# mehta-lab/VisCy

Hardware: AMD Instinct MI355X
Metric: training patches/sec (Z=5, 256x256, 1->2ch UNeXt2) (higher is better)
Workload: dtype bf16; 1 GPU; UNeXt2 2.5D convnextv2_tiny Z=5 256x256 1->2ch, fwd+MixedLoss(0.5,0,0.5)+bwd+AdamW; per_gpu_batch=512, global_batch=512, parallelism=dp1

## Files before the change

### include/vsx.h

```cpp
#ifndef VSX_H
#define VSX_H
#include <stddef.h>
#include <stdint.h>

#ifdef __cplusplus
extern "C" {
#endif

typedef void* vsx_stream_t;

#define VSX_F32 0
#define VSX_BF16 1

int32_t vsx_version(void);
const char* vsx_last_error(void);
const char* vsx_last_kernel(void);
int32_t vsx_set_flag(const char* name, int32_t value);
int32_t vsx_get_flag(const char* name);
int32_t vsx_det_workspace(float* ws, int64_t floats);
int32_t vsx_det_scope(int32_t on);
int32_t vsx_det_active(void);

#define VSX_A_ROWS 0
#define VSX_A_PATCH2 1
// ... 13 lines not shown
typedef struct VsxGemm {
  const void* A;
  const void* B;
  void* C;
  int32_t M, N, K;
  int32_t lda, ldb, ldc;
  int32_t a_mode, gh, gw, cs;
  int32_t nz;
  int32_t a_coff[8];
  int32_t b_off[8];
  int32_t c_coff[8];
  int32_t c_mode;
  int32_t c_cs;
  int32_t pro;
  const float* grn_s;
  const float* grn_b;
  int32_t hw;
  int32_t epi;
  const float* bias;
  const void* res;
  int32_t ldr;
  const void* aux;
  int32_t ldx;
  float* red0;
  float* red1;
  float* colsum;
  void* C2;
  int64_t b_bstride;
  const float* rscale;
} VsxGemm;

int32_t vsx_gemm_nt(const VsxGemm* p, int32_t dtype, vsx_stream_t stream);
int32_t vsx_gemm_nt_ln_bwd_supported(int64_t M, int32_t N, int32_t K, int32_t dtype);
int32_t vsx_gemm_tn(const VsxGemm* p, int32_t dtype, vsx_stream_t stream);

typedef struct VsxGemmPlan {
  const char* family;
  int32_t esize;
  int32_t tile[2];
  int32_t step;
  int32_t nbuf;
  int32_t pro_kind;
  int32_t tr;
  int32_t epi;
  int32_t grid[3], block;
  int32_t pro_bits;
  int64_t zero_c, zero_colsum;
  int64_t det_floats;
} VsxGemmPlan;
#define VSX_GEMM_NT 0
#define VSX_GEMM_TN 1
int32_t vsx_gemm_plan(int32_t kind, const VsxGemm* p, int32_t dtype, VsxGemmPlan* out);



int32_t vsx_dwconv7_fwd(const void* x, const float* w, const float* bias, const void* add, void* y,
    int32_t B, int32_t H, int32_t W, int32_t C, int32_t dtype, vsx_stream_t stream);

int32_t vsx_dwconv7_bwd_data(const void* dy, const float* w, const void* add, void* dx, int32_t B, int32_t H,
    int32_t W, int32_t C, int32_t dtype, vsx_stream_t stream);

int32_t vsx_dwconv7_bwd_weight(const void* dy, const void* x, float* dw, float* db, float* ws,
    int32_t ws_rows, int32_t B, int32_t H, int32_t W, int32_t C, int32_t dtype, vsx_stream_t stream);

int32_t vsx_head_conv_supported(int32_t H2, int32_t W2, int32_t c3, int32_t cmid, int32_t zo, int32_t dtype);
int64_t vsx_head_conv_det_floats(int32_t B, int32_t H2, int32_t W2);
// ... 354 lines not shown
```

### viscy_amd/_lib.py

```python

from __future__ import annotations

import ctypes as C
import os

import torch

_HERE = os.path.dirname(os.path.abspath(__file__))
LIB_PATH = os.environ.get("VSX_LIB", os.path.join(_HERE, "libvsx.so"))

VSX_F32, VSX_BF16 = 0, 1
A_ROWS, A_PATCH2, A_CONV3 = 0, 1, 2
PRO_NONE, PRO_GRN = 0, 1
EPI_NONE, EPI_BIAS, EPI_BIAS_GELU_SQ, EPI_BIAS_RES, EPI_DZ, EPI_BIAS_STATS, EPI_LN_BWD = 0, 1, 2, 3, 4, 5, 6
LOSS_SLOTS, LOSS_SLOT_STRIDE = 64, 32
SPOTLIGHT_CHUNK = 16384
SPOTLIGHT_THRESHOLD, SPOTLIGHT_MASK_U8, SPOTLIGHT_MASK_F32 = 0, 1, 2
SPOTLIGHT_WS_FWD, SPOTLIGHT_WS_OTSU = 0, 1

_I32, _F32, _P, _I64 = C.c_int32, C.c_float, C.c_void_p, C.c_int64


class VsxGemm(C.Structure):
    _fields_ = [
# ... 15 lines not shown
        ("rscale", _P),
    ]


class VsxGemmPlan(C.Structure):
    _fields_ = [
        ("family", C.c_char_p), ("esize", _I32), ("tile", _I32 * 2), ("step", _I32), ("nbuf", _I32), ("pro_kind", _I32), ("tr", _I32),
        ("epi", _I32), ("grid", _I32 * 3), ("block", _I32), ("pro_bits", _I32), ("zero_c", _I64), ("zero_colsum", _I64),
        ("det_floats", _I64),
    ]


class VsxWTask(C.Structure):
    _fields_ = [("kind", _I32), ("dtype", _I32), ("i0", _I32), ("i1", _I32), ("i2", _I32), ("i3", _I32),
                ("p0", _P), ("p1", _P), ("p2", _P), ("p3", _P), ("p4", _P), ("p5", _P), ("p6", _P), ("p7", _P)]


WTASK_PREP, WTASK_TRANSPOSE, WTASK_MATVEC, WTASK_MLP_PACK, WTASK_UNPREP, WTASK_MATVEC_T, WTASK_REDUCE_ROWS = 0, 1, 2, 3, 4, 5, 6

_SIGS = {
    "vsx_version": (_I32, []),
    "vsx_weight_tasks": (_I32, [_P, _I32, _P]),
    "vsx_last_error": (C.c_char_p, []),
    "vsx_last_kernel": (C.c_char_p, []),
    "vsx_set_flag": (_I32, [C.c_char_p, _I32]),
    "vsx_get_flag": (_I32, [C.c_char_p]),
    "vsx_det_workspace": (_I32, [_P, _I64]),
    "vsx_det_scope": (_I32, [_I32]),
    "vsx_det_active": (_I32, []),
    "vsx_gemm_nt": (_I32, [C.POINTER(VsxGemm), _I32, _P]),
    "vsx_gemm_tn": (_I32, [C.POINTER(VsxGemm), _I32, _P]),
    "vsx_gemm_plan": (_I32, [_I32, C.POINTER(VsxGemm), _I32, C.POINTER(VsxGemmPlan)]),
    "vsx_gemm_nt_ln_bwd_supported": (_I32, [_I64, _I32, _I32, _I32]),
    "vsx_ln_fwd": (_I32, [_P, _P, _P, _P, _P, _P, _I32, _I32, _F32, _I32, _P]),
    "vsx_ln_bwd": (_I32, [_P, _P, _P, _P, _P, _P, _P, _P, _P, _I32, _I32, _I32, _P]),
    "vsx_grn_scale": (_I32, [_P, _P, _P, _I32, _I32, _F32, _P]),
    "vsx_grn_bwd_stats": (_I32, [_P, _P, _P, _P, _P, _P, _P, _P, _I32, _I32, _F32, _P]),
    "vsx_grn_gelu_bwd": (_I32, [_P, _P, _P, _P, _P, _P, _I32, _I32, _I32, _I32, _I32, _P]),
    "vsx_dwconv7_fwd": (_I32, [_P, _P, _P, _P, _P, _I32, _I32, _I32, _I32, _I32, _P]),
    "vsx_dwconv7_bwd_data": (_I32, [_P, _P, _P, _P, _I32, _I32, _I32, _I32, _I32, _P]),
    "vsx_dwconv7_bwd_weight": (_I32, [_P, _P, _P, _P, _P, _I32, _I32, _I32, _I32, _I32, _I32, _P]),
    "vsx_stem_im2col": (_I32, [_P, _P, _P, _P, _I32, _I32, _I32, _I32, _I32, _I32, _I32, _I32, _I32, _P]),
    "vsx_stem_im2col_ld": (_I32, [_P, _P, _P, _P, _I32, _I32, _I32, _I32, _I32, _I32, _I32, _I32, _I32, _I32, _P]),
    "vsx_pad_cols": (_I32, [_P, _P, _I32, _I32, _I32, _I32, _P]),
    "vsx_im2col3x3": (_I32, [_P, _P, _I32, _I32, _I32, _I32, _I32, _P]),
    "vsx_col2im3x3": (_I32, [_P, _P, _I32, _I32, _I32, _I32, _I32, _P]),
    "vsx_pixel_shuffle_cat_fwd": (_I32, [_P, _P, _P, _I32, _I32, _I32, _I32, _I32, _I32, _P]),
    "vsx_pixel_shuffle_cat_bwd": (_I32, [_P, _P, _P, _I32, _I32, _I32, _I32, _I32, _I32, _P]),
    "vsx_head_shuffle_fwd": (_I32, [_P, _P, _I32, _I32, _I32, _I32, _I32, _I32, _I32, _P]),
    "vsx_head_shuffle_bwd": (_I32, [_P, _P, _I32, _I32, _I32, _I32, _I32, _I32, _I32, _P]),
    "vsx_head_out_fwd": (_I32, [_P] * 7 + [_I32] * 6 + [_F32, _I32, _P]),
    "vsx_head_out_bwd1": (_I32, [_P] * 11 + [_I32] * 6 + [_F32, _I32, _P]),
    "vsx_head_out_bwd1_wgrad": (_I32, [_P] * 13 + [_I32] * 6 + [_F32, _I32, _P]),
    "vsx_head_out_bwd2": (_I32, [_P] * 9 + [_I32] * 6 + [_F32, _I32, _P]),
    "vsx_loss_pool": (_I32, [_P] * 7 + [_I32] * 3 + [_P]),
    "vsx_ssim_scale_fwd": (_I32, [_P] * 5 + [_I32] * 5 + [_P]),
    "vsx_ssim_scale_bwd": (_I32, [_P] * 7 + [_I32] * 5 + [_F32, _F32, _P, _I32, _P]),
    "vsx_loss_finalize": (_I32, [_P] * 5 + [_F32, _I32, _I32, _I32, _F32, _F32, _F32, _P, _P, _P, _P, _P]),
    "vsx_ssim_scale_fwd_dmu": (_I32, [_P] * 6 + [_I32] * 6 + [_P]),
    "vsx_ssim_scale_bwd_in": (_I32, [_P] * 6 + [_I32] * 5 + [_F32, _F32, _P, _I32, _I32, _P]),
    "vsx_loss_tmax": (_I32, [_P, _I64, _P, _P]),
    "vsx_ssim_scale_fwd_fused": (_I32, [_P] * 11 + [_I32] * 6 + [_P]),
    "vsx_adamw": (_I32, [_P, _P, _P, _P, _P, _I64, _P]),
    "vsx_adamw_advance": (_I32, [_P, _P, _P, _P]),
    "vsx_fill_f32": (_I32, [_P, _I64, _F32, _P]),
    "vsx_mlp_supported": (_I32, [_I32, _I32, _I64, _I32]),
# ... 163 lines not shown
```

### viscy_amd/csrc/gemm.hip

```cpp
#include "vsx_common.h"
#include "../../include/vsx.h"

typedef __attribute__((ext_vector_type(4))) float f32x4;
typedef __attribute__((ext_vector_type(8))) __bf16 bf16x8;
typedef __attribute__((ext_vector_type(4))) short s16x4;

bool vsx_gemm_nt2_ok(const VsxGemm* p);
bool vsx_gemm_nt2_lnbwd_ok(const VsxGemm* p);
void vsx_gemm_nt2_plan(const VsxGemm* p, VsxGemmPlan& pl);
int vsx_gemm_nt2_run(const VsxGemmPlan& pl, const VsxGemm* p, hipStream_t s);

struct RowCoord {
  int b, y, x;
  bool valid;
};

__device__ __forceinline__ RowCoord decode_row(const VsxGemm& p, int m) {
  RowCoord r;
  r.valid = m < p.M;
  int mm = r.valid ? m : 0;
  if (p.a_mode == VSX_A_ROWS && p.c_mode == VSX_A_ROWS) {
    r.b = p.hw > 0 ? mm / p.hw : 0;
    r.y = 0;
    r.x = mm;
// ... 830 lines not shown
  NT_FAST2(T, VSX_EPI_BIAS_RES, BK, NBUF) NT_FAST2(T, VSX_EPI_DZ, BK, NBUF)
  switch (inst_key(pl)) {
    NT_GEN(bf16_t, 128, 2, 2, 128)
    NT_GEN(bf16_t, 128, 2, 2, 32) NT_GEN(float, 128, 2, 2, 32)
    NT_GEN(bf16_t, 64, 2, 2, 32) NT_GEN(float, 64, 2, 2, 32)
    NT_GEN(bf16_t, 32, 4, 1, 32) NT_GEN(float, 32, 4, 1, 32)
    NT_GEN(bf16_t, 16, 4, 1, 32) NT_GEN(float, 16, 4, 1, 32)
    NT_FAST(bf16_t, 64, 1)
    NT_FAST(bf16_t, 64, 2)
    NT_FAST(bf16_t, 32, 1)
    NT_FAST(bf16_t, 32, 2) NT_FAST(float, 32, 2)
    default: vsx_set_error("vsx_gemm_nt: the plan names no instantiation"); return 1;
  }
#undef NT_GEN
#undef NT_FAST1
#undef NT_FAST2
#undef NT_FAST
  VSX_LAUNCH_CHECK();
  g_vsx_last_kernel = pl.family;
  return 0;
}

extern "C" int32_t vsx_gemm_nt(const VsxGemm* p, int32_t dtype, vsx_stream_t stream) {
  VsxGemmPlan pl;
  if (int e = plan_nt(p, dtype, pl)) return e;
  return run_nt(pl, p, reinterpret_cast<hipStream_t>(stream));
}

extern "C" int32_t vsx_gemm_nt_ln_bwd_supported(int64_t M, int32_t N, int32_t K, int32_t dtype) {
  if (dtype != VSX_BF16 || M <= 0 || M >= (1ll << 31)) return 0;
  VsxGemm q = {};
  q.M = (int32_t)M; q.N = N; q.K = K; q.lda = K; q.ldb = K; q.ldc = N; q.a_mode = VSX_A_ROWS; q.c_mode = VSX_A_ROWS; q.epi = VSX_EPI_LN_BWD;
  return vsx_gemm_nt2_lnbwd_ok(&q) ? 1 : 0;
}

template <bool TR>
__device__ __forceinline__ bf16x8 lds_frag_mn_bf16(const char* tile, int LDB, int col0, int p16, int kq) {
  if (TR) {
    const int q = p16;
    const char* a0 = tile + (kq * 4 + (q >> 2)) * LDB + (col0 + (q & 3) * 4) * 2;
    const char* a1 = a0 + 16 * LDB;
    s16x4 lo = __builtin_amdgcn_ds_read_tr16_b64_v4i16((s16x4 __attribute__((address_space(3)))*)(a0));
    s16x4 hi = __builtin_amdgcn_ds_read_tr16_b64_v4i16((s16x4 __attribute__((address_space(3)))*)(a1));
    union {
      struct { s16x4 lo, hi; } s;
      bf16x8 v;
    } u;
    u.s.lo = lo;
    u.s.hi = hi;
    return u.v;
  } else {
    union {
      unsigned short h[8];
      bf16x8 v;
    } u;
#pragma unroll
    for (int j = 0; j < 8; ++j) {
      int mloc = j < 4 ? kq * 4 + j : 16 + kq * 4 + (j - 4);
      u.h[j] = *reinterpret_cast<const unsigned short*>(tile + mloc * LDB + (col0 + p16) * 2);
    }
    return u.v;
  }
}

template <typename T, bool TR>
__device__ __forceinline__ typename Frag<T>::type lds_frag_mn(const char* tile, int LDB, int col0, int p16, int kq,
// ... 666 lines not shown
```

### viscy_amd/csrc/gemm_nt2.hip

```cpp
#include "vsx_common.h"
#include "../../include/vsx.h"

typedef __attribute__((ext_vector_type(4))) float nt2_f32x4;
typedef __attribute__((ext_vector_type(8))) __bf16 nt2_bf16x8;

namespace {

constexpr int BM = 256, BK = 32, NST = 3;
constexpr int ROWB = BK * 2;
constexpr int CW_LD = 68;
constexpr int CW_BYTES = 16 * CW_LD * 4;
constexpr int RED_OFF = 8 * CW_BYTES;

template <int BN>
struct Nt2Geom {
  static constexpr int FN = BN / 32;
  static constexpr int A_BYTES = BM * ROWB, B_BYTES = BN * ROWB, STAGE = A_BYTES + B_BYTES;
  static constexpr int NPA = (BM / 16) / 8, NPB = (BN / 16) / 8;
  static constexpr int PER_SLAB = NPA + NPB;
  static constexpr int LDS_BYTES = NST * STAGE;
  static constexpr int WAVES_PER_SIMD = BN == 128 ? 4 : 2;
  static_assert(RED_OFF + 8 * 2 * (BN / 2) * 4 <= LDS_BYTES, "epilogue staging overlays the operand stages");
};

template <int EPI, int BN, bool PRO = false>
__global__ __launch_bounds__(512, Nt2Geom<BN>::WAVES_PER_SIMD) void gemm_nt2_kernel(const VsxGemm p) {
  typedef Nt2Geom<BN> G;
  constexpr int FN = G::FN, A_BYTES = G::A_BYTES, STAGE = G::STAGE, WN = BN / 2;
  constexpr int PRO_FLOATS = PRO ? 2 * 3072 : 4;
  __shared__ __attribute__((aligned(1024))) char smem[G::LDS_BYTES];
  __shared__ __attribute__((aligned(16))) float gsb[PRO_FLOATS];
  const int tid = threadIdx.x, lane = tid & 63;
  const int wave = __builtin_amdgcn_readfirstlane(tid >> 6);
  const int wm = wave >> 1, wn = wave & 1;
// ... 261 lines not shown
    }
  }

  if constexpr (REDUCE) {
    if (p.hw % BM == 0) {
      asm volatile("s_waitcnt lgkmcnt(0)" ::: "memory");
      __builtin_amdgcn_s_barrier();
      if (tid < BN && n0 + tid < p.N) {
        const int w0 = tid / WN, c = tid % WN;
        float a0 = 0.f, a1 = 0.f;
#pragma unroll
        for (int w = 0; w < 4; ++w) {
          a0 += red[((w * 2 + w0) * 2 + 0) * WN + c];
          if constexpr (EPI == VSX_EPI_DZ) a1 += red[((w * 2 + w0) * 2 + 1) * WN + c];
        }
        if (EPI == VSX_EPI_BIAS_GELU_SQ && p.aux != nullptr) {
          reinterpret_cast<float*>(const_cast<void*>(p.aux))[(size_t)tile_m * p.N + n0 + tid] = a0;
        } else {
          atomicAdd(p.red0 + (size_t)b_tile * p.N + n0 + tid, a0);
          if constexpr (EPI == VSX_EPI_DZ) atomicAdd(p.red1 + (size_t)b_tile * p.N + n0 + tid, a1);
        }
      }
    }
  }
}

#ifdef NT2_TS
__device__ unsigned long long g_nt2_ts[8 * 80];
#define NT2_STAMP(k) do { if (blockIdx.x == gridDim.x / 2 + 3 && lane == 0) g_nt2_ts[wave * 80 + (k)] = __builtin_amdgcn_s_memtime(); } while (0)
#else
#define NT2_STAMP(k) do { } while (0)
#endif

template <int BN>
__global__ __launch_bounds__(512, 2) void gemm_nt2_lnbwd_kernel(const VsxGemm p) {
  typedef Nt2Geom<BN> G;
  constexpr int FN = BN / 16, A_BYTES = G::A_BYTES, STAGE = G::STAGE, NCG = BN / 64;
  __shared__ __attribute__((aligned(1024))) char smem[G::LDS_BYTES];
  const int tid = threadIdx.x, lane = tid & 63;
  const int wave = __builtin_amdgcn_readfirstlane(tid >> 6);
  const int p16 = lane & 15, kq = lane >> 4;
  int bid = blockIdx.x;
  const int m0 = bid * BM;
  NT2_STAMP(0);

  const int dr = lane >> 2;
  const int dc = (lane & 3) ^ ((lane >> 4) & 2);
  const char* Ab = reinterpret_cast<const char*>(p.A) + (size_t)m0 * (size_t)p.lda * 2;
  const char* Bb = reinterpret_cast<const char*>(p.B);
  uint32_t offA[G::NPA], offB[G::NPB];
#pragma unroll
  for (int i = 0; i < G::NPA; ++i) offA[i] = (uint32_t)((wave + 8 * i) * 16 + dr) * (uint32_t)(p.lda * 2) + dc * 16;
#pragma unroll
  for (int i = 0; i < G::NPB; ++i) {
    int nb = (wave + 8 * i) * 16 + dr;
    nb = nb < p.N ? nb : p.N - 1;
    offB[i] = (uint32_t)nb * (uint32_t)(p.ldb * 2) + dc * 16;
  }
  auto issue = [&](int kt, int st) {
    char* S = smem + st * STAGE;
    const char* Ak = Ab + (size_t)kt * ROWB;
    const char* Bk = Bb + (size_t)kt * ROWB;
#pragma unroll
    for (int i = 0; i < G::NPA; ++i)
      __builtin_amdgcn_global_load_lds((const __attribute__((address_space(1))) void*)(Ak + offA[i]),
                                       (__attribute__((address_space(3))) void*)(S + (wave + 8 * i) * 1024), 16, 0, 0);
#pragma unroll
    for (int i = 0; i < G::NPB; ++i)
      __builtin_amdgcn_global_load_lds((const __attribute__((address_space(1))) void*)(Bk + offB[i]),
                                       (__attribute__((address_space(3))) void*)(S + A_BYTES + (wave + 8 * i) * 1024), 16, 0, 0);
// ... 16 lines not shown
    for (int jg = 0; jg < FN; jg += 4) {
      nt2_bf16x8 bf[4];
#pragma unroll
      for (int j = 0; j < 4; ++j) bf[j] = *reinterpret_cast<const nt2_bf16x8*>(S + fragB + (jg + j) * 16 * ROWB);
#pragma unroll
      for (int i = 0; i < 2; ++i)
#pragma unroll
        for (int j = 0; j < 4; ++j)
          acc[i][jg + j] = __builtin_amdgcn_mfma_f32_16x16x32_bf16(af[i], bf[j], acc[i][jg + j], 0, 0, 0);
    }
  };

  const int nk = p.K / BK;
  constexpr int er_ = 0;
  const int erow = lane >> 3, ecol = (lane & 7) * 8;
  const bf16_t* XHp = reinterpret_cast<const bf16_t*>(p.aux);
  uint4 xpre[2][NCG][2];
  float mupre[2][2], rspre[2][2];
  auto prefetch_pass = [&](int i) {
#pragma unroll
    for (int h = 0; h < 2; ++h) {
      const int m = m0 + wave * 32 + i * 16 + erow + 8 * h;
      mupre[i][h] = p.grn_b ? p.grn_b[m] : 0.f;
      rspre[i][h] = p.grn_s[m];
#pragma unroll
      for (int cg = 0; cg < NCG; ++cg) {
        const int n = cg * 64 + ecol;
        xpre[i][cg][h] = n < p.N ? ldvec<bf16_t>(XHp + (size_t)m * p.ldx + n) : make_uint4(0u, 0u, 0u, 0u);
      }
    }
  };
  auto prefetch_rows = [&]() { prefetch_pass(0); };
  (void)er_;
  issue(0, 0);
  if (nk > 1) issue(1, 1);
  if (nk < 3) prefetch_rows();
  int st = 0, stn = NST - 1;
  for (int kt = 0; kt < nk; ++kt) {
    if (kt + 1 < nk) {
      if constexpr (G::PER_SLAB == 3) asm volatile("s_waitcnt vmcnt(3)" ::: "memory");
      else asm volatile("s_waitcnt vmcnt(4)" ::: "memory");
    } else {
      asm volatile("s_waitcnt vmcnt(0)" ::: "memory");
    }
    __builtin_amdgcn_s_barrier();
    if (kt < 64) NT2_STAMP(8 + kt);
    if (kt + 2 < nk) issue(kt + 2, stn);
    if (kt == nk - 3) prefetch_rows();
    compute(st);
    st = st == NST - 1 ? 0 : st + 1;
    stn = stn == NST - 1 ? 0 : stn + 1;
  }
  NT2_STAMP(1);
  asm volatile("s_waitcnt lgkmcnt(0)" ::: "memory");
  __builtin_amdgcn_s_barrier();
  NT2_STAMP(2);

  float* Cw = reinterpret_cast<float*>(smem + wave * CW_BYTES);
  const int er = lane >> 3, ec = (lane & 7) * 8;
  const float invC = 1.f / (float)p.N;
  const bf16_t* XH = reinterpret_cast<const bf16_t*>(p.aux);
  bf16_t* DY = reinterpret_cast<bf16_t*>(p.C);
  const float* MEAN = p.grn_b;
#pragma unroll
  for (int i = 0; i < 2; ++i) {
    float v[NCG][2][8];
    uint4 (&xq)[NCG][2] = xpre[i];
    float s1[2] = {0.f, 0.f}, s2[2] = {0.f, 0.f};
#pragma unroll
    for (int cg = 0; cg < NCG; ++cg) {
      const int n = cg * 64 + ec;
      const bool ok = n < p.N;
#pragma unroll
      for (int j = 0; j < 4; ++j)
#pragma unroll
        for (int r = 0; r < 4; ++r) Cw[(kq * 4 + r) * CW_LD + j * 16 + p16] = acc[i][cg * 4 + j][r];
      __builtin_amdgcn_fence(__ATOMIC_RELEASE, "wavefront");
      __builtin_amdgcn_wave_barrier();
#pragma unroll
      for (int h = 0; h < 2; ++h) {
        const float4 t0 = *reinterpret_cast<const float4*>(Cw + (er + 8 * h) * CW_LD + ec);
        const float4 t1 = *reinterpret_cast<const float4*>(Cw + (er + 8 * h) * CW_LD + ec + 4);
        const float t[8] = {t0.x, t0.y, t0.z, t0.w, t1.x, t1.y, t1.z, t1.w};
        float xf[8];
        unpack<bf16_t>(xq[cg][h], xf);
        if (MEAN && ok) {
          const float mu = mupre[i][h], rsd = rspre[i][h];
#pragma unroll
          for (int e = 0; e < 8; ++e) xf[e] = (xf[e] - mu) * rsd;
          xq[cg][h] = pack<bf16_t>(xf);
          unpack<bf16_t>(xq[cg][h], xf);
        }
#pragma unroll
        for (int e = 0; e < 8; ++e) {
          const float d = ok ? round_bf16(t[e]) : 0.f;
          v[cg][h][e] = d;
          s1[h] += d;
          s2[h] = fmaf(d, xf[e], s2[h]);
        }
      }
      __builtin_amdgcn_fence(__ATOMIC_RELEASE, "wavefront");
      __builtin_amdgcn_wave_barrier();
    }
    NT2_STAMP(3 + i);
    if (i == 0) prefetch_pass(1);
#pragma unroll
    for (int h = 0; h < 2; ++h) {
      s1[h] += __shfl_xor(s1[h], 1, 64); s1[h] += __shfl_xor(s1[h], 2, 64); s1[h] += __shfl_xor(s1[h], 4, 64);
      s2[h] += __shfl_xor(s2[h], 1, 64); s2[h] += __shfl_xor(s2[h], 2, 64); s2[h] += __shfl_xor(s2[h], 4, 64);
      const int m = m0 + wave * 32 + i * 16 + er + 8 * h;
      const float rs = MEAN ? 1.f : rspre[i][h];
      const float m1 = s1[h] * invC, m2 = s2[h] * invC;
#pragma unroll
      for (int cg = 0; cg < NCG; ++cg) {
        const int n = cg * 64 + ec;
        if (n < p.N) {
          float xf[8], o[8];
          unpack<bf16_t>(xq[cg][h], xf);
#pragma unroll
          for (int e = 0; e < 8; ++e) o[e] = rs * (v[cg][h][e] - m1 - xf[e] * m2);
          stvec<bf16_t>(DY + (size_t)m * p.ldc + n, pack<bf16_t>(o));
        }
      }
    }
  }
  NT2_STAMP(5);
}

int pick_bn(int N) {
  if (g_vsx_nt2 & 4) return 128;
  int best = 128, best_cost = 1 << 30;
  for (int bn = 128; bn <= ((g_vsx_nt2 & 8) ? 256 : 384); bn += 128) {
    const int tiles = (N + bn - 1) / bn;
    if (3 * (tiles * bn - N) > N && bn != 128) continue;
    const int cost = tiles * (BM + bn);
    if (cost < best_cost) { best_cost = cost; best = bn; }
  }
  return best;
}

}

bool vsx_gemm_nt2_lnbwd_ok(const VsxGemm* p) {
  return p->a_mode == VSX_A_ROWS && p->c_mode == VSX_A_ROWS && p->pro == VSX_PRO_NONE && p->nz <= 1 && p->K % BK == 0 &&
         p->M % BM == 0 && p->N >= 64 && p->N <= 256 && p->N % 8 == 0 && p->b_bstride == 0 &&
         (unsigned long long)BM * p->lda * 2 < (1ull << 32) && (unsigned long long)p->N * p->ldb * 2 < (1ull << 32);
}

bool vsx_gemm_nt2_ok(const VsxGemm* p) {
  if (p->epi == VSX_EPI_LN_BWD) return vsx_gemm_nt2_lnbwd_ok(p);
  if (!(g_vsx_nt2 & 1)) return false;
  if (p->a_mode != VSX_A_ROWS || p->c_mode != VSX_A_ROWS || p->nz > 1) return false;
  if (p->pro != VSX_PRO_NONE) {
    if (p->pro != VSX_PRO_GRN || p->hw <= 0 || p->hw % BM != 0 || p->K > 3072) return false;
    if (p->epi != VSX_EPI_BIAS_RES && p->epi != VSX_EPI_NONE) return false;
  }
// ... 7 lines not shown
  if (g_vsx_nt2 & 2) return true;
  if (vsx_det_on() && p->epi == VSX_EPI_BIAS_GELU_SQ) return true;
  const int bn = pick_bn(p->N);
  if ((long)(p->M / BM) * vsx_cdiv(p->N, bn) < 256) return false;
  if (p->epi == VSX_EPI_DZ) return false;
  if (p->pro == VSX_PRO_GRN) return p->K >= 768 && p->N >= 192;
  if (p->epi == VSX_EPI_BIAS_GELU_SQ) return bn == 384 && p->N % 384 == 0 && p->K >= 384 && p->K <= 768;
  return p->K >= 768 && (p->N > 192 || ((g_vsx_nt2 & 16) && p->N == 192));
}

void vsx_gemm_nt2_plan(const VsxGemm* p, VsxGemmPlan& pl) {
  const bool lnbwd = p->epi == VSX_EPI_LN_BWD;
  const int bn = lnbwd ? (p->N <= 128 ? 128 : 256) : pick_bn(p->N);
  pl.family = "gemm_nt2";
  pl.tile[0] = BM; pl.tile[1] = bn; pl.step = BK; pl.nbuf = NST;
  pl.epi = p->epi;
  pl.pro_kind = p->pro == VSX_PRO_GRN;
  pl.grid[0] = (p->M / BM) * (lnbwd ? 1 : vsx_cdiv(p->N, bn)); pl.grid[1] = pl.grid[2] = 1;
  pl.block = 512;
  if (vsx_det_on() && p->epi == VSX_EPI_BIAS_GELU_SQ && p->hw > 0 && p->hw % BM == 0 && p->hw > BM) pl.det_floats = (long)(p->M / BM) * p->N;
}

int vsx_gemm_nt2_run(const VsxGemmPlan& pl, const VsxGemm* p, hipStream_t s) {
  VsxGemm q = *p;
  float* det_ws;
  if (int e = vsx_det_take("vsx_gemm_nt", pl.det_floats, &det_ws)) return e;
  if (det_ws) q.aux = det_ws;
  const dim3 grid(pl.grid[0]), block(pl.block);
#define NT2(EPI, BN, PRO) case (EPI) << 12 | (BN) << 1 | (PRO): hipLaunchKernelGGL((gemm_nt2_kernel<EPI, BN, PRO>), grid, block, 0, s, q); break;
#define NT2_BN(BN)  \
  NT2(VSX_EPI_NONE, BN, false) NT2(VSX_EPI_BIAS, BN, false) NT2(VSX_EPI_BIAS_GELU_SQ, BN, false) NT2(VSX_EPI_BIAS_RES, BN, false) \
  NT2(VSX_EPI_DZ, BN, false) NT2(VSX_EPI_NONE, BN, true) NT2(VSX_EPI_BIAS_RES, BN, true)
#define NT2_LNBWD(BN) case VSX_EPI_LN_BWD << 12 | (BN) << 1: hipLaunchKernelGGL((gemm_nt2_lnbwd_kernel<BN>), grid, block, 0, s, q); break;
  switch (pl.epi << 12 | pl.tile[1] << 1 | pl.pro_kind) {
    NT2_BN(128)
    NT2_BN(256)
    NT2_BN(384)
    NT2_LNBWD(128)
    NT2_LNBWD(256)
    default: vsx_set_error("vsx_gemm_nt: the plan names no gemm_nt2 instantiation"); return 1;
  }
#undef NT2
#undef NT2_BN
#undef NT2_LNBWD
  VSX_LAUNCH_CHECK();
  g_vsx_last_kernel = pl.family;
  if (det_ws) return vsx_det_group_sum(det_ws, p->N, 0, p->red0, p->M / p->hw, p->hw / BM, p->N, s);
  return 0;
}

#ifdef NT2_TS
extern "C" int32_t vsx_debug_nt2_ts(unsigned long long* host_out) {
  return hipMemcpyFromSymbol(host_out, HIP_SYMBOL(g_nt2_ts), sizeof(g_nt2_ts)) == hipSuccess ? 0 : 1;
}
#endif
```

### viscy_amd/engine_unext2.py

```python

from __future__ import annotations

import os
from collections import namedtuple
from typing import NamedTuple

import torch
from torch import Tensor

from . import _lib as L
from . import ops as hip_ops
from .flat import FlatEngine, engine_apply


class _BlockW:

    __slots__ = ("C", "p", "dw_w", "W1f", "W1fT", "b1f", "W2", "W2T", "v1", "fc2_w", "fc2_b", "grn_w", "grn_b", "dp", "img", "img2", "b2f")


class _ProjW:
    __slots__ = ("cin", "cout", "taps", "ln", "conv", "W", "WT")


FWD_UNFUSED, FWD_PAIR, FWD_FC1 = 0, 1, 2
# ... 740 lines not shown
            B, H, Wd = sv["shape"]
            dev = self.device
            za_key = ("bwd", B, H, Wd, sv["masked"])
            self._za = za = _ZeroArena(dev, self._za_need.get(za_key, 0), self.ops)
            if cfg.get("head") == "embed":
                d = self._embed_tail_bwd(sv, dout[0], dout[1], dt, B)
            elif cfg.get("head", "conv") == "shuffle":
                fh, fw = sv["head"]
                sxy = cfg["stem_kernel"][-1]
                vs = o.voxel_shuffle_bwd
                if (cfg["out_channels"] * cfg["out_stack_depth"] * sxy * sxy) % (8 if dt == torch.bfloat16 else 4):
                    vs = o.narrow_voxel_shuffle_bwd
                d = vs(dout.contiguous().float(), B, fh, fw, cfg["out_channels"], cfg["out_stack_depth"], sxy, True, dt)
            else:
                hdt = self._head_dtype(dt)
                d = self._head_conv_bwd(sv, dout, hdt, B, dev)
                if hdt != dt:
                    d = d.to(dt)
            dskips = {}
            for k in (2, 1, 0) if cfg.get("head") != "embed" else ():
                proj, blocks = W["dec"][k]
                st_sv = sv["dec"][k]
                cat, xn, mean, rstd, c_up, sc = st_sv["proj"]
                _, sh, sw_, _ = (None, *sv["feat_dims"][2 - k])
                Mk, ccat = B * sh * sw_, c_up + sc
                for bw, bsv in zip(reversed(blocks), reversed(st_sv["blocks"])):
                    d = self._block_bwd(d, bw, bsv, B, sh, sw_, dt)
                if proj.cout < 16:
                    dxn = o.narrow_proj_bwd(d, cat, mean, rstd, proj.ln.weight, proj.ln.bias, proj.conv.weight, g(proj.conv.weight),
                                            g(proj.conv.bias), Mk, ccat, proj.cout)
                else:
                    o.gemm("tn", xn, d, g(proj.conv.weight), Mk, proj.cout, ccat, ccat, proj.cout, ccat, dtype=dt,
                           colsum=g(proj.conv.bias))
                    dxn = torch.empty((Mk, ccat), dtype=dt, device=dev)
                    o.gemm("nt", d, proj.WT, dxn, Mk, ccat, proj.cout, proj.cout, proj.cout, ccat, dtype=dt)
                dcat = o.ln_bwd(dxn, cat, mean, rstd, proj.ln.weight, None, g(proj.ln.weight), g(proj.ln.bias), Mk, ccat)
                del dxn
                d, dskips[2 - k] = o.pixel_shuffle_cat_bwd(dcat, B, sh // 2, sw_ // 2, c_up, sc)
                del dcat
                pre = W["dec_pre"][k]
                if pre is not None:
                    pc, _, WpT = pre
                    lh, lw, cpc = sh // 2, sw_ // 2, 4 * c_up
                    Ml = B * lh * lw
                    col = o.im2col3x3(st_sv["pre_in"], B, lh, lw, cpc)
                    dWp = self._za.take(cpc, 9 * cpc)
                    o.gemm("tn", col, d, dWp, Ml, cpc, 9 * cpc, 9 * cpc, cpc, 9 * cpc, dtype=dt, colsum=g(pc.bias))
                    o.unprep_grad(dWp, g(pc.weight), cpc, cpc, 9)
                    del col
                    dcol = torch.empty((Ml, 9 * cpc), dtype=dt, device=dev)
                    o.gemm("nt", d, WpT, dcol, Ml, 9 * cpc, cpc, cpc, cpc, 9 * cpc, dtype=dt)
                    d = o.col2im3x3(dcol, B, lh, lw, cpc)
                    del dcol
            yield from self._segment_end(0)
            if self.encoder_frozen():
                self._za_need[za_key] = za.used
                yield from self._segment_end(1)
                yield from self._segment_end(2)
                return
            for i in (3, 2, 1, 0):
                proj, blocks = W["enc"][i]
                st_sv = sv["enc"][i]
                ch, cw, cc = sv["feat_dims"][i]
                for bw, bsv in zip(reversed(blocks), reversed(st_sv["blocks"])):
                    d = self._block_bwd(d, bw, bsv, B, ch, cw, dt)
                if proj is not None:
                    prev, xn, mean, rstd = st_sv["proj"]
                    cin = proj.cin
                    Mo = B * ch * cw
# ... 49 lines not shown
```

### viscy_amd/ops.py

```python

from __future__ import annotations

import contextlib
import ctypes as C
import os
import threading
from typing import Sequence

import torch
from torch import Tensor

from . import _lib as L
from ._lib import VsxGemm, VsxGemmPlan, check, dtype_code, lib, ptr, stream


class Scratch:

    def __init__(self, alloc=None):
        self._alloc = alloc or (lambda floats, dev: torch.empty(floats, dtype=torch.float32, device=dev))
        self._tls = threading.local()
        self.held: list = []

    def take(self, dev, floats: int):
        arenas = getattr(self._tls, "arenas", None)
# ... 98 lines not shown
    p.grn_s, p.grn_b = ptr(grn_s), ptr(grn_b)
    p.hw = hw
    p.epi = epi
    p.bias, p.res, p.ldr = ptr(bias), ptr(res), ldr
    p.aux, p.ldx = ptr(aux), ldx
    p.red0, p.red1, p.colsum = ptr(red0), ptr(red1), ptr(colsum)
    p.C2 = ptr(C2)
    p.b_bstride = b_bstride
    p.rscale = ptr(rscale)
    if plan is not None:
        return check(lib().vsx_gemm_plan(0 if kind == "nt" else 1, C.byref(p), dtype_code(dtype), C.byref(plan)), f"gemm_plan_{kind}")
    if kind == "nt" and epi == L.EPI_BIAS_GELU_SQ:
        _det(A.device, lambda: _gemm_det_floats(p, dtype))
    fn = lib().vsx_gemm_nt if kind == "nt" else lib().vsx_gemm_tn
    check(fn(C.byref(p), dtype_code(dtype), stream()), f"gemm_{kind}")


def _gemm_det_floats(p: VsxGemm, dtype: torch.dtype) -> int:
    plan = VsxGemmPlan()
    check(lib().vsx_gemm_plan(0, C.byref(p), dtype_code(dtype), C.byref(plan)), "gemm_plan_nt")
    return plan.det_floats


def tn_grn_stats_ok(M: int, N: int, K: int, hw: int, dtype: torch.dtype) -> bool:
    if dtype != torch.bfloat16 or not lib().vsx_get_flag(b"tn_rect") & 8:
        return False
    p = VsxGemm()
    p.A = p.B = p.C = p.grn_s = p.grn_b = p.aux = p.red0 = 1
    p.M, p.N, p.K, p.lda, p.ldb, p.ldc, p.ldx, p.nz, p.pro, p.hw = M, N, K, K, N, K, K, 1, L.PRO_GRN, hw
    return lib().vsx_gemm_plan(1, C.byref(p), L.VSX_BF16, C.byref(VsxGemmPlan())) == 0


def dgrad_ln_bwd(dh: Tensor, WT: Tensor, xh: Tensor, rstd: Tensor, M: int, C: int, K: int,
                 mean: Tensor | None = None) -> Tensor | None:
    if dh.dtype != torch.bfloat16 or not lib().vsx_gemm_nt_ln_bwd_supported(M, C, K, dtype_code(dh.dtype)):
        return None
    dy = torch.empty((M, C), dtype=dh.dtype, device=dh.device)
    gemm("nt", dh, WT, dy, M, C, K, K, K, C, dtype=dh.dtype, epi=L.EPI_LN_BWD, aux=xh, ldx=C, grn_s=rstd, grn_b=mean)
    return dy


def gemm_z(kind: str, *args, nz: int, a_coff, b_off, c_coff, **kw) -> None:
    for s in range(0, nz, 8):
        e = min(nz, s + 8)
        gemm(kind, *args, nz=e - s, a_coff=a_coff[s:e], b_off=b_off[s:e], c_coff=c_coff[s:e], **kw)


def ln_fwd(x: Tensor, gamma: Tensor | None, beta: Tensor | None, rows: int, Cc: int, eps: float = 1e-6,
           need_mean: bool = True):
    y = torch.empty_like(x)
    mean = torch.empty(rows, dtype=torch.float32, device=x.device) if need_mean else None
    rstd = torch.empty(rows, dtype=torch.float32, device=x.device)
    check(lib().vsx_ln_fwd(ptr(x), ptr(y), ptr(mean), ptr(rstd), ptr(gamma), ptr(beta), rows, Cc, eps,
                           dtype_code(x.dtype), stream()), "ln_fwd")
    return y, mean, rstd


def ln_bwd(dy: Tensor, x: Tensor, mean: Tensor | None, rstd: Tensor, gamma: Tensor | None, add: Tensor | None,
           dgamma: Tensor | None, dbeta: Tensor | None, rows: int, Cc: int) -> Tensor:
    dx = torch.empty_like(dy)
    check(lib().vsx_ln_bwd(ptr(dy), ptr(x), ptr(mean), ptr(rstd), ptr(gamma), ptr(add), ptr(dx), ptr(dgamma),
                           ptr(dbeta), rows, Cc, dtype_code(dy.dtype), stream()), "ln_bwd")
    return dx


def grn_scale(colsq: Tensor, gamma: Tensor, eps: float = 1e-6) -> Tensor:
    s = torch.empty_like(colsq)
    check(lib().vsx_grn_scale(ptr(colsq), ptr(gamma), ptr(s), colsq.shape[0], colsq.shape[1], eps, stream()), "grn_scale")
    return s


# ... 1010 lines not shown
```

Measured before the change: 5600 patches/s.

## Fuse affine LayerNorm backward into decoder projection dgrad GEMM epilogue

Adds an affine variant of the NT GEMM LN-backward epilogue that applies gamma, computes the input gradient, and accumulates per-tile dgamma/dbeta partials into a workspace. A row-reduction kernel (or the deterministic group sum) then finishes the partials. The decoder projection backward uses it, avoiding a round trip of the dxn intermediate through memory and a separate ln_bwd launch. In exchange it adds register pressure and LDS staging in the epilogue, two extra small reduction launches, and it falls back to the old path when the shape is unsupported.

```diff
diff --git a/include/vsx.h b/include/vsx.h
--- a/include/vsx.h
+++ b/include/vsx.h
@@ -69,6 +69,7 @@
 
 int32_t vsx_gemm_nt(const VsxGemm* p, int32_t dtype, vsx_stream_t stream);
 int32_t vsx_gemm_nt_ln_bwd_supported(int64_t M, int32_t N, int32_t K, int32_t dtype);
+int64_t vsx_gemm_nt_ln_bwd_affine_ws_floats(int64_t M, int32_t N, int32_t K, int32_t dtype);
 int32_t vsx_gemm_tn(const VsxGemm* p, int32_t dtype, vsx_stream_t stream);
 
 typedef struct VsxGemmPlan {
diff --git a/viscy_amd/_lib.py b/viscy_amd/_lib.py
--- a/viscy_amd/_lib.py
+++ b/viscy_amd/_lib.py
@@ -71,6 +71,7 @@
     "vsx_gemm_tn": (_I32, [C.POINTER(VsxGemm), _I32, _P]),
     "vsx_gemm_plan": (_I32, [_I32, C.POINTER(VsxGemm), _I32, C.POINTER(VsxGemmPlan)]),
     "vsx_gemm_nt_ln_bwd_supported": (_I32, [_I64, _I32, _I32, _I32]),
+    "vsx_gemm_nt_ln_bwd_affine_ws_floats": (_I64, [_I64, _I32, _I32, _I32]),
     "vsx_ln_fwd": (_I32, [_P, _P, _P, _P, _P, _P, _I32, _I32, _F32, _I32, _P]),
     "vsx_ln_bwd": (_I32, [_P, _P, _P, _P, _P, _P, _P, _P, _P, _I32, _I32, _I32, _P]),
     "vsx_grn_scale": (_I32, [_P, _P, _P, _I32, _I32, _F32, _P]),
diff --git a/viscy_amd/csrc/gemm.hip b/viscy_amd/csrc/gemm.hip
--- a/viscy_amd/csrc/gemm.hip
+++ b/viscy_amd/csrc/gemm.hip
@@ -886,6 +886,10 @@
   VsxGemm q = {};
   q.M = (int32_t)M; q.N = N; q.K = K; q.lda = K; q.ldb = K; q.ldc = N; q.a_mode = VSX_A_ROWS; q.c_mode = VSX_A_ROWS; q.epi = VSX_EPI_LN_BWD;
   return vsx_gemm_nt2_lnbwd_ok(&q) ? 1 : 0;
+}
+
+extern "C" int64_t vsx_gemm_nt_ln_bwd_affine_ws_floats(int64_t M, int32_t N, int32_t K, int32_t dtype) {
+  return vsx_gemm_nt_ln_bwd_supported(M, N, K, dtype) ? 2 * (M / 256) * (int64_t)N : 0;
 }
 
 template <bool TR>
diff --git a/viscy_amd/csrc/gemm_nt2.hip b/viscy_amd/csrc/gemm_nt2.hip
--- a/viscy_amd/csrc/gemm_nt2.hip
+++ b/viscy_amd/csrc/gemm_nt2.hip
@@ -1,5 +1,7 @@
 #include "vsx_common.h"
 #include "../../include/vsx.h"
+
+__global__ void reduce_rows_kernel(const float* __restrict__ ws, float* __restrict__ out, int R, int N);
 
 typedef __attribute__((ext_vector_type(4))) float nt2_f32x4;
 typedef __attribute__((ext_vector_type(8))) __bf16 nt2_bf16x8;
@@ -327,10 +329,12 @@
 #define NT2_STAMP(k) do { } while (0)
 #endif
 
-template <int BN>
+template <int BN, int NCG = BN / 64, bool AFF = false>
 __global__ __launch_bounds__(512, 2) void gemm_nt2_lnbwd_kernel(const VsxGemm p) {
   typedef Nt2Geom<BN> G;
-  constexpr int FN = BN / 16, A_BYTES = G::A_BYTES, STAGE = G::STAGE, NCG = BN / 64;
+  constexpr int FN = NCG * 4, A_BYTES = G::A_BYTES, STAGE = G::STAGE;
+  constexpr int GAM_OFF = RED_OFF + 8 * 2 * BN * 4;
+  static_assert(GAM_OFF + BN * 4 <= G::LDS_BYTES, "the affine epilogue's staging overlays the operand stages");
   __shared__ __attribute__((aligned(1024))) char smem[G::LDS_BYTES];
   const int tid = threadIdx.x, lane = tid & 63;
   const int wave = __builtin_amdgcn_readfirstlane(tid >> 6);
@@ -413,6 +417,8 @@
   };
   auto prefetch_rows = [&]() { prefetch_pass(0); };
   (void)er_;
+  float gpre = 1.f;
+  if constexpr (AFF) if (tid < p.N) gpre = p.bias[tid];
   issue(0, 0);
   if (nk > 1) issue(1, 1);
   if (nk < 3) prefetch_rows();
@@ -436,6 +442,11 @@
   asm volatile("s_waitcnt lgkmcnt(0)" ::: "memory");
   __builtin_amdgcn_s_barrier();
   NT2_STAMP(2);
+  float* gam = reinterpret_cast<float*>(smem + GAM_OFF);
+  if constexpr (AFF) {
+    if (tid < BN) gam[tid] = gpre;
+    __syncthreads();
+  }
 
   float* Cw = reinterpret_cast<float*>(smem + wave * CW_BYTES);
   const int er = lane >> 3, ec = (lane & 7) * 8;
@@ -443,15 +454,27 @@
   const bf16_t* XH = reinterpret_cast<const bf16_t*>(p.aux);
   bf16_t* DY = reinterpret_cast<bf16_t*>(p.C);
   const float* MEAN = p.grn_b;
+  float* red = reinterpret_cast<float*>(smem + RED_OFF);
 #pragma unroll
   for (int i = 0; i < 2; ++i) {
-    float v[NCG][2][8];
+    float v[AFF ? 1 : NCG][2][8];
+    uint4 vq[AFF ? NCG : 1][2];
     uint4 (&xq)[NCG][2] = xpre[i];
     float s1[2] = {0.f, 0.f}, s2[2] = {0.f, 0.f};
+    auto load_gamma = [&](int n, float (&gm)[8]) {
+      const float4 g0 = *reinterpret_cast<const float4*>(gam + n), g1 = *reinterpret_cast<const float4*>(gam + n + 4);
+      gm[0] = g0.x; gm[1] = g0.y; gm[2] = g0.z; gm[3] = g0.w; gm[4] = g1.x; gm[5] = g1.y; gm[6] = g1.z; gm[7] = g1.w;
+    };
 #pragma unroll
     for (int cg = 0; cg < NCG; ++cg) {
       const int n = cg * 64 + ec;
       const bool ok = n < p.N;
+      float gm[8], pg[8], pb[8];
+      if constexpr (AFF) {
+        load_gamma(n, gm);
+#pragma unroll
+        for (int e = 0; e < 8; ++e) { pg[e] = 0.f; pb[e] = 0.f; }
+      }
 #pragma unroll
       for (int j = 0; j < 4; ++j)
 #pragma unroll
@@ -464,45 +487,114 @@
         const float4 t1 = *reinterpret_cast<const float4*>(Cw + (er + 8 * h) * CW_LD + ec + 4);
         const float t[8] = {t0.x, t0.y, t0.z, t0.w, t1.x, t1.y, t1.z, t1.w};
         float xf[8];
+        if constexpr (AFF) asm volatile("" : "+v"(xq[cg][h].x), "+v"(xq[cg][h].y), "+v"(xq[cg][h].z), "+v"(xq[cg][h].w));
         unpack<bf16_t>(xq[cg][h], xf);
-        if (MEAN && ok) {
+        if constexpr (AFF) {
+          const float mu = mupre[i][h], rsd = rspre[i][h];
+#pragma unroll
+          for (int e = 0; e < 8; ++e) xf[e] = ok ? (xf[e] - mu) * rsd : 0.f;
+        } else if (MEAN && ok) {
           const float mu = mupre[i][h], rsd = rspre[i][h];
 #pragma unroll
           for (int e = 0; e < 8; ++e) xf[e] = (xf[e] - mu) * rsd;
           xq[cg][h] = pack<bf16_t>(xf);
           unpack<bf16_t>(xq[cg][h], xf);
         }
+        float dq[8];
 #pragma unroll
         for (int e = 0; e < 8; ++e) {
-          const float d = ok ? round_bf16(t[e]) : 0.f;
-          v[cg][h][e] = d;
+          float d = ok ? round_bf16(t[e]) : 0.f;
+          if constexpr (AFF) {
+            pg[e] = fmaf(d, xf[e], pg[e]);
+            pb[e] += d;
+            dq[e] = d;
+            d *= gm[e];
+          } else {
+            v[cg][h][e] = d;
+          }
           s1[h] += d;
           s2[h] = fmaf(d, xf[e], s2[h]);
         }
+        if constexpr (AFF) vq[cg][h] = pack<bf16_t>(dq);
       }
       __builtin_amdgcn_fence(__ATOMIC_RELEASE, "wavefront");
       __builtin_amdgcn_wave_barrier();
+      if constexpr (AFF) {
+        float* Pg = Cw + (er * 2) * CW_LD + ec;
+        *reinterpret_cast<float4*>(Pg) = make_float4(pg[0], pg[1], pg[2], pg[3]);
+        *reinterpret_cast<float4*>(Pg + 4) = make_float4(pg[4], pg[5], pg[6], pg[7]);
+        *reinterpret_cast<float4*>(Pg + CW_LD) = make_float4(pb[0], pb[1], pb[2], pb[3]);
+        *reinterpret_cast<float4*>(Pg + CW_LD + 4) = make_float4(pb[4], pb[5], pb[6], pb[7]);
+        __builtin_amdgcn_fence(__ATOMIC_RELEASE, "wavefront");
+        __builtin_amdgcn_wave_barrier();
+        float a0 = 0.f, a1 = 0.f;
+#pragma unroll
+        for (int r = 0; r < 8; ++r) {
+          a0 += Cw[(r * 2) * CW_LD + lane];
+          a1 += Cw[(r * 2 + 1) * CW_LD + lane];
+        }
+        float* rw = red + (wave * 2) * BN + cg * 64 + lane;
+        if (i == 0) { rw[0] = a0; rw[BN] = a1; }
+        else { rw[0] += a0; rw[BN] += a1; }
+        __builtin_amdgcn_fence(__ATOMIC_RELEASE, "wavefront");
+        __builtin_amdgcn_wave_barrier();
+      }
     }
     NT2_STAMP(3 + i);
-    if (i == 0) prefetch_pass(1);
+    if constexpr (AFF) {
+#pragma unroll
+      for (int cg = 0; cg < NCG; ++cg)
+#pragma unroll
+        for (int h = 0; h < 2; ++h) {
+          asm volatile("" : "+v"(xq[cg][h].x), "+v"(xq[cg][h].y), "+v"(xq[cg][h].z), "+v"(xq[cg][h].w));
+          asm volatile("" : "+v"(vq[cg][h].x), "+v"(vq[cg][h].y), "+v"(vq[cg][h].z), "+v"(vq[cg][h].w));
+        }
+    }
+    constexpr bool LATE_PRE = AFF && NCG == 4;
+    if (i == 0 && !LATE_PRE) prefetch_pass(1);
 #pragma unroll
     for (int h = 0; h < 2; ++h) {
       s1[h] += __shfl_xor(s1[h], 1, 64); s1[h] += __shfl_xor(s1[h], 2, 64); s1[h] += __shfl_xor(s1[h], 4, 64);
       s2[h] += __shfl_xor(s2[h], 1, 64); s2[h] += __shfl_xor(s2[h], 2, 64); s2[h] += __shfl_xor(s2[h], 4, 64);
       const int m = m0 + wave * 32 + i * 16 + er + 8 * h;
-      const float rs = MEAN ? 1.f : rspre[i][h];
-      const float m1 = s1[h] * invC, m2 = s2[h] * invC;
+      const float rs = (MEAN && !AFF) ? 1.f : rspre[i][h];
+      const float m1 = AFF ? s1[h] / (float)p.N : s1[h] * invC, m2 = AFF ? s2[h] / (float)p.N : s2[h] * invC;
 #pragma unroll
       for (int cg = 0; cg < NCG; ++cg) {
         const int n = cg * 64 + ec;
         if (n < p.N) {
           float xf[8], o[8];
           unpack<bf16_t>(xq[cg][h], xf);
-#pragma unroll
-          for (int e = 0; e < 8; ++e) o[e] = rs * (v[cg][h][e] - m1 - xf[e] * m2);
+          if constexpr (AFF) {
+            const float mu = mupre[i][h];
+            float gm[8], df[8];
+            load_gamma(n, gm);
+            unpack<bf16_t>(vq[cg][h], df);
+#pragma unroll
+            for (int e = 0; e < 8; ++e) o[e] = rs * (df[e] * gm[e] - m1 - ((xf[e] - mu) * rs) * m2);
+          } else {
+#pragma unroll
+            for (int e = 0; e < 8; ++e) o[e] = rs * (v[cg][h][e] - m1 - xf[e] * m2);
+          }
           stvec<bf16_t>(DY + (size_t)m * p.ldc + n, pack<bf16_t>(o));
         }
       }
+    }
+    if (i == 0 && LATE_PRE) prefetch_pass(1);
+  }
+  if constexpr (AFF) {
+    __syncthreads();
+    if (tid < p.N) {
+      float a0 = 0.f, a1 = 0.f;
+#pragma unroll
+      for (int w = 0; w < 8; ++w) {
+        a0 += red[(w * 2 + 0) * BN + tid];
+        a1 += red[(w * 2 + 1) * BN + tid];
+      }
+      const size_t tiles = (size_t)(p.M / BM);
+      float* ws = reinterpret_cast<float*>(p.C2);
+      ws[(size_t)bid * p.N + tid] = a0;
+      ws[(tiles + (size_t)bid) * p.N + tid] = a1;
     }
   }
   NT2_STAMP(5);
@@ -576,19 +668,40 @@
   NT2(VSX_EPI_NONE, BN, false) NT2(VSX_EPI_BIAS, BN, false) NT2(VSX_EPI_BIAS_GELU_SQ, BN, false) NT2(VSX_EPI_BIAS_RES, BN, false) \
   NT2(VSX_EPI_DZ, BN, false) NT2(VSX_EPI_NONE, BN, true) NT2(VSX_EPI_BIAS_RES, BN, true)
 #define NT2_LNBWD(BN) case VSX_EPI_LN_BWD << 12 | (BN) << 1: hipLaunchKernelGGL((gemm_nt2_lnbwd_kernel<BN>), grid, block, 0, s, q); break;
-  switch (pl.epi << 12 | pl.tile[1] << 1 | pl.pro_kind) {
+#define NT2_LNAFF(BN, NCG) case 1 << 20 | (NCG) << 16 | VSX_EPI_LN_BWD << 12 | (BN) << 1: \
+    hipLaunchKernelGGL((gemm_nt2_lnbwd_kernel<BN, NCG, true>), grid, block, 0, s, q); break;
+  const bool ln_aff = pl.epi == VSX_EPI_LN_BWD && p->bias != nullptr;
+  if (ln_aff)
+    VSX_CHECK(p->grn_b && p->red0 && p->red1 && p->C2,
+              "vsx_gemm_nt: EPI_LN_BWD with an affine (bias = gamma) needs grn_b = mean, red0 = dgamma, red1 = dbeta and the "
+              "workspace C2 (vsx_gemm_nt_ln_bwd_affine_ws_floats)");
+  switch ((ln_aff ? 1 << 20 | vsx_cdiv(p->N, 64) << 16 : 0) | pl.epi << 12 | pl.tile[1] << 1 | pl.pro_kind) {
     NT2_BN(128)
     NT2_BN(256)
     NT2_BN(384)
     NT2_LNBWD(128)
     NT2_LNBWD(256)
+    NT2_LNAFF(128, 1) NT2_LNAFF(128, 2) NT2_LNAFF(256, 3) NT2_LNAFF(256, 4)
     default: vsx_set_error("vsx_gemm_nt: the plan names no gemm_nt2 instantiation"); return 1;
   }
 #undef NT2
 #undef NT2_BN
 #undef NT2_LNBWD
+#undef NT2_LNAFF
   VSX_LAUNCH_CHECK();
   g_vsx_last_kernel = pl.family;
+  if (ln_aff) {
+    const int R = p->M / BM;
+    const float* ws = reinterpret_cast<const float*>(p->C2);
+    if (vsx_det_on()) {
+      if (int e = vsx_det_group_sum(ws, p->N, 0, p->red0, 1, R, p->N, s)) return e;
+      return vsx_det_group_sum(ws + (size_t)R * p->N, p->N, 0, p->red1, 1, R, p->N, s);
+    }
+    const dim3 rg(vsx_cdiv(p->N, 64), vsx_cdiv(R, 64));
+    hipLaunchKernelGGL(reduce_rows_kernel, rg, dim3(256), 0, s, ws, p->red0, R, p->N);
+    hipLaunchKernelGGL(reduce_rows_kernel, rg, dim3(256), 0, s, ws + (size_t)R * p->N, p->red1, R, p->N);
+    VSX_LAUNCH_CHECK();
+  }
   if (det_ws) return vsx_det_group_sum(det_ws, p->N, 0, p->red0, p->M / p->hw, p->hw / BM, p->N, s);
   return 0;
 }
diff --git a/viscy_amd/engine_unext2.py b/viscy_amd/engine_unext2.py
--- a/viscy_amd/engine_unext2.py
+++ b/viscy_amd/engine_unext2.py
@@ -796,9 +796,14 @@
                 else:
                     o.gemm("tn", xn, d, g(proj.conv.weight), Mk, proj.cout, ccat, ccat, proj.cout, ccat, dtype=dt,
                            colsum=g(proj.conv.bias))
-                    dxn = torch.empty((Mk, ccat), dtype=dt, device=dev)
-                    o.gemm("nt", d, proj.WT, dxn, Mk, ccat, proj.cout, proj.cout, proj.cout, ccat, dtype=dt)
-                dcat = o.ln_bwd(dxn, cat, mean, rstd, proj.ln.weight, None, g(proj.ln.weight), g(proj.ln.bias), Mk, ccat)
+                    dcat = o.dgrad_ln_bwd(d, proj.WT, cat, rstd, Mk, ccat, proj.cout, mean=mean, gamma=proj.ln.weight,
+                                          dgamma=g(proj.ln.weight), dbeta=g(proj.ln.bias)) if self._hip else None
+                    dxn = None
+                    if dcat is None:
+                        dxn = torch.empty((Mk, ccat), dtype=dt, device=dev)
+                        o.gemm("nt", d, proj.WT, dxn, Mk, ccat, proj.cout, proj.cout, proj.cout, ccat, dtype=dt)
+                if dxn is not None:
+                    dcat = o.ln_bwd(dxn, cat, mean, rstd, proj.ln.weight, None, g(proj.ln.weight), g(proj.ln.bias), Mk, ccat)
                 del dxn
                 d, dskips[2 - k] = o.pixel_shuffle_cat_bwd(dcat, B, sh // 2, sw_ // 2, c_up, sc)
                 del dcat
diff --git a/viscy_amd/ops.py b/viscy_amd/ops.py
--- a/viscy_amd/ops.py
+++ b/viscy_amd/ops.py
@@ -154,11 +154,24 @@
 
 
 def dgrad_ln_bwd(dh: Tensor, WT: Tensor, xh: Tensor, rstd: Tensor, M: int, C: int, K: int,
-                 mean: Tensor | None = None) -> Tensor | None:
-    if dh.dtype != torch.bfloat16 or not lib().vsx_gemm_nt_ln_bwd_supported(M, C, K, dtype_code(dh.dtype)):
+                 mean: Tensor | None = None, gamma: Tensor | None = None, dgamma: Tensor | None = None,
+                 dbeta: Tensor | None = None) -> Tensor | None:
+    if dh.dtype != torch.bfloat16:
+        return None
+    if gamma is None:
+        if not lib().vsx_gemm_nt_ln_bwd_supported(M, C, K, dtype_code(dh.dtype)):
+            return None
+        dy = torch.empty((M, C), dtype=dh.dtype, device=dh.device)
+        gemm("nt", dh, WT, dy, M, C, K, K, K, C, dtype=dh.dtype, epi=L.EPI_LN_BWD, aux=xh, ldx=C, grn_s=rstd, grn_b=mean)
+        return dy
+    if mean is None or dgamma is None or dbeta is None:
+        raise ValueError("dgrad_ln_bwd: the affine form needs mean, dgamma and dbeta")
+    floats = lib().vsx_gemm_nt_ln_bwd_affine_ws_floats(M, C, K, dtype_code(dh.dtype))
+    if floats <= 0:
         return None
     dy = torch.empty((M, C), dtype=dh.dtype, device=dh.device)
-    gemm("nt", dh, WT, dy, M, C, K, K, K, C, dtype=dh.dtype, epi=L.EPI_LN_BWD, aux=xh, ldx=C, grn_s=rstd, grn_b=mean)
+    gemm("nt", dh, WT, dy, M, C, K, K, K, C, dtype=dh.dtype, epi=L.EPI_LN_BWD, aux=xh, ldx=C, grn_s=rstd, grn_b=mean,
+         bias=gamma, red0=dgamma, red1=dbeta, C2=_workspace(dh.device, floats))
     return dy
 
 
```

Measured after the change: 5597 patches/s. Within noise of the previous version (-0.1%).
